# Gaukler/PlainRenderer

Hardware: AMD Instinct MI355X
Metric: frames/sec full GI+shade+post @4K; %HBM roofline; 1/2/4/8-GPU scaling (higher is better)
Workload: dtype f32

## Files before the change

include/plr.h:

```cpp
#ifndef PLR_H
#define PLR_H
#include <stddef.h>
#include <stdint.h>
#ifdef __cplusplus
extern "C" {
#endif

#define PLR_OK 0
#define PLR_ERR_INVALID_ARGUMENT (-1)
#define PLR_ERR_HIP (-2)
#define PLR_ERR_UNKNOWN_SHADER (-3)
#define PLR_ERR_BINDING (-4)
#define PLR_ERR_NOT_INITIALISED (-5)
#define PLR_ERR_UNSUPPORTED (-6)

#define PLR_INVALID_INDEX 0xFFFFFFFFu

enum plr_image_type { PLR_IMAGE_1D = 0, PLR_IMAGE_2D = 1, PLR_IMAGE_3D = 2, PLR_IMAGE_CUBE = 3 };
enum plr_mip_count { PLR_MIP_ONE = 0, PLR_MIP_FULL_CHAIN = 1, PLR_MIP_MANUAL = 2, PLR_MIP_FULL_CHAIN_ALREADY_IN_DATA = 3 };
enum plr_image_usage { PLR_USAGE_STORAGE = 1, PLR_USAGE_SAMPLED = 2, PLR_USAGE_ATTACHMENT = 4 };
enum plr_image_format {
    PLR_FORMAT_R8 = 0, PLR_FORMAT_RG8, PLR_FORMAT_RGBA8, PLR_FORMAT_R16_SFLOAT, PLR_FORMAT_RG16_SFLOAT,
    PLR_FORMAT_RG32_SFLOAT, PLR_FORMAT_RG16_SNORM, PLR_FORMAT_RGBA16_SFLOAT, PLR_FORMAT_RGBA16_SNORM,
    PLR_FORMAT_RGBA32_SFLOAT, PLR_FORMAT_R11G11B10_UFLOAT, PLR_FORMAT_DEPTH16, PLR_FORMAT_DEPTH32,
// ... 126 lines not shown
int plr_replay_frame(uint32_t count, float* out_total_gpu_ms);
int plr_upload_image(plr_image_handle image, uint32_t mip_level, const void* data, size_t size);
int plr_upload_image_rows(plr_image_handle image, uint32_t mip_level, uint32_t row_begin, uint32_t row_count, const void* data, size_t size);
int plr_download_image(plr_image_handle image, uint32_t mip_level, void* out_data, size_t size);
int plr_download_storage_buffer(plr_storage_buffer_handle buffer, void* out_data, size_t offset, size_t size);
int plr_download_uniform_buffer(plr_uniform_buffer_handle buffer, void* out_data, size_t offset, size_t size);
int plr_get_image_device_pointer(plr_image_handle image, uint32_t mip_level, void** out_ptr, size_t* out_size);
int plr_get_storage_buffer_device_pointer(plr_storage_buffer_handle buffer, void** out_ptr, size_t* out_size);
int plr_get_stream(void** out_hip_stream);
int plr_get_launch_stream(void** out_hip_stream);
int plr_copy_device_memory(void* dst, const void* src, size_t size);
int plr_copy_device_memory_2d(void* dst, size_t dst_pitch, const void* src, size_t src_pitch, size_t width_bytes, size_t rows);
int plr_read_device_memory(void* dst_host, const void* src, size_t size);
int plr_write_device_memory(void* dst, const void* src_host, size_t size);
int plr_get_supported_shaders(const char** out_names, uint32_t capacity);
int plr_debug_math_eval(int fn, const float* a, const float* b, float* out, int64_t n);
int plr_debug_codec_eval(int fn, const void* in, void* out, int64_t n);
int plr_debug_set_decision_signature(size_t words);
int plr_debug_read_decision_signature(uint32_t* out_words, size_t words);
int plr_debug_verify_histogram_thresholds(float min_luminance, float max_luminance, uint64_t* out_mismatches);
int plr_debug_verify_r11g11b10_fast(uint64_t* out4);
int plr_debug_sky_lut_eval(plr_image_handle sky_lut, const float* directions, float* out_rgb, int64_t n);
int plr_debug_pcf_tap_table(float* out_xy, size_t floats);
int plr_debug_sampler_eval(plr_image_handle image, uint32_t mip_level, int filter, int address, const float* coords, float* out, int64_t n);

#ifdef __cplusplus
}
#endif
#endif
```

plainrenderer_amd/backend.py:

```python
import ctypes as C
import os
import struct
from dataclasses import dataclass, field
from enum import IntEnum
from typing import List, Optional, Sequence

import numpy as np

_HERE = os.path.dirname(os.path.abspath(__file__))
LIB_PATH = os.environ.get("PLR_LIB") or os.path.join(_HERE, "libplr.so")


class PlrError(RuntimeError):
    pass


class ImageType(IntEnum):
    Type1D = 0
    Type2D = 1
    Type3D = 2
    TypeCube = 3


class MipCount(IntEnum):
# ... 163 lines not shown

def spec_int(location, v):
    return SpecialisationConstant(location, struct.pack("<i", int(v)))


def spec_uint(location, v):
    return SpecialisationConstant(location, struct.pack("<I", int(v)))


def spec_float(location, v):
    return SpecialisationConstant(location, struct.pack("<f", float(v)))


def _load():
    if not os.path.exists(LIB_PATH):
        raise PlrError("HIP backend library missing: %s (run `python -c 'import __graft_entry__ as g; g.build()'`). "
                       "There is no CPU fallback." % LIB_PATH)
    lib = C.CDLL(LIB_PATH)
    lib.plr_last_error.restype = C.c_char_p
    return lib


EXPORTED_SYMBOLS = [
    "plr_debug_pcf_tap_table", "plr_setup", "plr_shutdown", "plr_recreate_swapchain", "plr_last_error", "plr_wait_for_gpu_idle", "plr_update_shader_code",
    "plr_resize_images", "plr_recreate_image", "plr_resize_storage_buffer", "plr_new_frame", "plr_set_compute_pass_execution", "plr_prepare_for_drawcall_recording",
    "plr_set_uniform_buffer_data", "plr_set_storage_buffer_data", "plr_set_global_descriptor_set_resources",
    "plr_update_compute_pass_shader_description", "plr_render_frame", "plr_get_image_global_texture_array_index",
    "plr_create_compute_pass", "plr_create_image", "plr_create_uniform_buffer", "plr_create_storage_buffer", "plr_create_sampler",
    "plr_create_temporary_image", "plr_get_swapchain_input_image", "plr_get_memory_stats", "plr_get_renderpass_timings",
    "plr_get_last_frame_cpu_time", "plr_get_image_description", "plr_set_pass_timing", "plr_get_last_frame_gpu_time",
    "plr_replay_frame", "plr_upload_image", "plr_download_image", "plr_download_storage_buffer", "plr_download_uniform_buffer",
    "plr_get_image_device_pointer", "plr_get_storage_buffer_device_pointer", "plr_get_stream", "plr_get_launch_stream", "plr_copy_device_memory", "plr_read_device_memory", "plr_write_device_memory", "plr_get_supported_shaders",
    "plr_debug_math_eval", "plr_debug_codec_eval", "plr_debug_sampler_eval", "plr_debug_sky_lut_eval", "plr_debug_verify_histogram_thresholds", "plr_debug_verify_r11g11b10_fast", "plr_debug_set_decision_signature", "plr_debug_read_decision_signature", "plr_set_math_mode", "plr_get_math_mode", "plr_set_stream_overlap", "plr_get_stream_overlap", "plr_set_pass_fusion", "plr_get_pass_fusion", "plr_set_pass_fusion_reorder", "plr_get_general_kernel_executions", "plr_get_edge_signal", "plr_set_async_tail", "plr_get_async_tail", "plr_set_early_parts", "plr_get_early_parts", "plr_set_host_callback_execution", "plr_set_host_callback_execution_on", "plr_upload_image_rows",
    "plr_copy_device_memory_2d", "plr_set_global_descriptor_set_layout",
]


class RenderBackend:

    def __init__(self, width, height, device=0):
        self.lib = _load()
        self._open = False
        self._check(self.lib.plr_setup(C.c_int(device), C.c_uint32(width), C.c_uint32(height)))
        self._open = True
        self.width, self.height = width, height

    def _check(self, rc):
# ... 246 lines not shown
        return p.value

    def debugMathEval(self, fn, a, b=None):
        a = np.ascontiguousarray(a, np.float32)
        out = np.empty_like(a)
        bp = None
        if b is not None:
            b = np.ascontiguousarray(b, np.float32)
            bp = b.ctypes.data_as(C.c_void_p)
        self._check(self.lib.plr_debug_math_eval(C.c_int(fn), a.ctypes.data_as(C.c_void_p), bp, out.ctypes.data_as(C.c_void_p), C.c_int64(a.size)))
        return out

    def debugSkyLutEval(self, sky_lut, directions):
        d = np.ascontiguousarray(directions, np.float32).reshape(-1, 3)
        out = np.empty_like(d)
        self._check(self.lib.plr_debug_sky_lut_eval(_ImageHandle(sky_lut.type, sky_lut.index), d.ctypes.data_as(C.c_void_p), out.ctypes.data_as(C.c_void_p), C.c_int64(d.shape[0])))
        return out

    def debugPcfTapTable(self):
        out = np.empty((256, 12, 2), np.float32)
        self._check(self.lib.plr_debug_pcf_tap_table(out.ctypes.data_as(C.c_void_p), C.c_size_t(out.size)))
        return out

    def debugVerifyHistogramThresholds(self, min_luminance, max_luminance):
        n = C.c_uint64()
        self._check(self.lib.plr_debug_verify_histogram_thresholds(C.c_float(min_luminance), C.c_float(max_luminance), C.byref(n)))
        return n.value

    def debugVerifyR11G11B10Fast(self):
        out = (C.c_uint64 * 4)()
        self._check(self.lib.plr_debug_verify_r11g11b10_fast(out))
        return tuple(int(v) for v in out)

    def setPassFusion(self, level):
        self._check(self.lib.plr_set_pass_fusion(C.c_int(int(level))))

    def setPassFusionReorder(self, enabled):
        self._check(self.lib.plr_set_pass_fusion_reorder(C.c_int(int(bool(enabled)))))

    def getPassFusion(self):
        e, n = C.c_int(), C.c_uint32()
        self._check(self.lib.plr_get_pass_fusion(C.byref(e), C.byref(n)))
        return e.value, n.value

    def getEdgeSignal(self):
        p, v = C.c_void_p(), C.c_uint32()
# ... 58 lines not shown
```

plainrenderer_amd/csrc/backend.cpp:

```cpp
#include "backend.h"
#include "kernels_fast/pcf_taps.h"

#include <dlfcn.h>
#include <deque>
#include <algorithm>
#include <chrono>
#include <mutex>
#include <cstdlib>
#include <atomic>
#include <set>
#include <thread>
#include <unordered_map>
#include <unordered_set>
#include <cmath>
#include <cstring>
#include <map>
#include <memory>

#include "../../include/plr.h"

namespace plr {

struct ShaderEntry { std::string name; LaunchFn fn = nullptr; LaunchFn fast = nullptr; };
static bool shaderReadsBindless(const std::string& shader) {
// ... 1985 lines not shown
}

int plr_debug_sky_lut_eval(plr_image_handle sky_lut, const float* directions, float* out_rgb, int64_t n) {
    NEED_INIT_JOINED();
    ImageRes* im = resolveImage(sky_lut);
    if (!im || !directions || !out_rgb || n <= 0) return setErr(PLR_ERR_INVALID_ARGUMENT, "plr_debug_sky_lut_eval: invalid argument");
    HIP_TRY(hipStreamSynchronize(g->stream));
    return launchSkyLutProbe(makeView(*im, 0), directions, out_rgb, n);
}

int plr_debug_pcf_tap_table(float* out_xy, size_t floats) {
    NEED_INIT_JOINED();
    if (!out_xy || floats != kPcfTapTableBytes / sizeof(float)) return setErr(PLR_ERR_INVALID_ARGUMENT, "plr_debug_pcf_tap_table: out_xy must hold 256 x 12 x 2 floats");
    void* table = nullptr;
    HIP_TRY(hipMalloc(&table, kPcfTapTableBytes));
    hipError_t e = buildPcfTapTable((float2*)table, g->stream);
    if (e == hipSuccess) e = hipStreamSynchronize(g->stream);
    if (e == hipSuccess) e = hipMemcpy(out_xy, table, kPcfTapTableBytes, hipMemcpyDeviceToHost);
    hipFree(table);
    HIP_TRY(e);
    return PLR_OK;
}

int plr_debug_sampler_eval(plr_image_handle image, uint32_t mip_level, int filter, int address, const float* coords, float* out, int64_t n) {
    NEED_INIT_JOINED();
    ImageRes* im = resolveImage(image);
    if (!im || mip_level >= im->mips.size()) return setErr(PLR_ERR_INVALID_ARGUMENT, "plr_debug_sampler_eval: invalid image handle or mip level");
    if (!coords || !out || n <= 0) return setErr(PLR_ERR_INVALID_ARGUMENT, "plr_debug_sampler_eval: null argument");
    HIP_TRY(hipStreamSynchronize(g->stream));
    return launchSamplerProbe(makeView(*im, mip_level), filter, address, coords, out, n);
}

int plr_set_math_mode(int mode) {
    NEED_INIT_JOINED();
    if (mode != PLR_MATH_EXACT && mode != PLR_MATH_FAST) return setErr(PLR_ERR_INVALID_ARGUMENT, "math mode must be PLR_MATH_EXACT or PLR_MATH_FAST");
    if (mode == PLR_MATH_EXACT) if (int rc = ensureExactSet()) return rc;
    g->mathMode = mode;
    return PLR_OK;
}
int plr_get_math_mode(int* out_mode) { NEED_INIT(); *out_mode = g->mathMode; return PLR_OK; }

int plr_set_pass_timing(int enabled) { NEED_INIT(); g->passTiming = enabled != 0; return PLR_OK; }

int plr_get_renderpass_timings(plr_renderpass_time* out_times, uint32_t* inout_count) {
    NEED_INIT();
    if (!inout_count) return setErr(PLR_ERR_INVALID_ARGUMENT, "inout_count is null");
// ... 136 lines not shown
```

plainrenderer_amd/csrc/kernels_fast/pcf_taps.h:

```cpp
#pragma once
#include <hip/hip_runtime.h>
#include <stdint.h>

namespace plr {

constexpr int kPcfTaps = 12, kPcfNoiseValues = 256;
constexpr size_t kPcfTapTableBytes = (size_t)kPcfNoiseValues * kPcfTaps * 2 * sizeof(float);

hipError_t buildPcfTapTable(float2* table, hipStream_t stream);

}
```

plainrenderer_amd/csrc/kernels_fast/shading_fast.hip:

```cpp
#include "../backend.h"
#include "../device/shading_common.h"
#include "../device/fastmath.h"
#include "../device/buffer_fetch.h"
#include "upscale_quad.h"
#include "pcf_taps.h"
#include <cstdlib>
#include <type_traits>
#include <map>

namespace plr {

namespace fastshade {

#ifndef PLR_SHADE_WAVES
#define PLR_SHADE_WAVES 5
#endif

PLR_DI float rcpf(float x) { return __builtin_amdgcn_rcpf(x); }
PLR_DI float rsqf(float x) { return __builtin_amdgcn_rsqf(x); }
PLR_DI float sqrtv(float x) { return __builtin_amdgcn_sqrtf(x); }
PLR_DI float fmin1(float a, float b) { return __builtin_fminf(a, b); }
PLR_DI float fmax1(float a, float b) { return __builtin_fmaxf(a, b); }
PLR_DI float fclamp(float x, float lo, float hi) { return __builtin_fminf(__builtin_fmaxf(x, lo), hi); }
PLR_DI float fmix(float a, float b, float t) { return a + (b - a) * t; }
// ... 118 lines not shown
    r = accumulateTexel(r, q1.z, q1.w, a2 * b);
    return r;
}

struct ShadeParams {
    ImgView color, depth, normal, albedo, specular, brdfLut, shadowMaps[4], ysh, cocg, volumetricLut, skyLut;
    const LightBuffer* light;
    const ShadowCascadeInfo* shadowInfo;
    const VolumetricLightingSettings* vol;
    const GlobalUbo* g;
    const ImgView* bindless;
    uint32_t bindlessCount;
    uint32_t cascadeCount;
    int coverW, coverH, yBase;
    int xBase;
    uint32_t* sig;
    ImgView noiseTex;
    const float4* pcfTaps;
    const float4* pcfTapsByPosition;
    uint32_t pcfPositions;
    const uint2* lutEnergyFootprint;
    const uint32_t* lutEnergyNonFinite;
    uint32_t skipUnlit;
};
PLR_DI float uniformValue(float x) { return u2f((uint32_t)__builtin_amdgcn_readfirstlane((int)f2u(x))); }
PLR_DI bool finiteBits(float x) { return (f2u(x) & 0x7f800000u) != 0x7f800000u; }

#define PLR_SHADE_UNIFORM_PARAMS const GlobalUbo* __restrict__ gUniform, const LightBuffer* __restrict__ lightUniform, const ShadowCascadeInfo* __restrict__ shadowUniform, \
                                 const VolumetricLightingSettings* __restrict__ volUniform
#define PLR_SHADE_ADOPT_UNIFORMS(P) do { (P).g = gUniform; (P).light = lightUniform; (P).shadowInfo = shadowUniform; (P).vol = volUniform; } while (0)
#define PLR_SHADE_UNIFORM_ARGS(P) (P).g, (P).light, (P).shadowInfo, (P).vol

struct PcfTapRow { float4 q[kPcfTaps / 2]; };
PLR_DI float calcShadow(vec3 pos, const ImgView& shadowMap, const float* __restrict__ m, float lssX, float lssY, const PcfTapRow& taps) {
    float cxy0, cxy1;
    uint32_t depthThreshold;
    {
#pragma clang fp contract(off)
        const float x = ((m[0] * pos.x + m[4] * pos.y) + m[8] * pos.z) + m[12];
        const float y = ((m[1] * pos.x + m[5] * pos.y) + m[9] * pos.z) + m[13];
        const float z = ((m[2] * pos.x + m[6] * pos.y) + m[10] * pos.z) + m[14];
        const float w = ((m[3] * pos.x + m[7] * pos.y) + m[11] * pos.z) + m[15];
        const float rw = rcpf(w);
        cxy0 = divRNr(x, w, rw) * 0.5f + 0.5f;
        cxy1 = divRNr(y, w, rw) * 0.5f + 0.5f;
        const float actualDepth = fclamp(divRNr(z, w, rw), 0.f, 1.f);
// ... 49 lines not shown
    if (MULTISCATTER == 0) {
        const float energyAverage = ReflectedEnergyAverage(r);
        const float energyIncoming = lutEnergy(P, r, NoL);
        const float unscaled = (1.f - energyIncoming) * (1.f - energyOutgoing) * rcpf(3.1415f * (1.f - energyAverage));
        const vec3 den = 1.f - fresnelAverage * (1.f - energyAverage);
        const vec3 scaling = (fresnelAverage * fresnelAverage * energyAverage) * vec3(rcpf(den.x), rcpf(den.y), rcpf(den.z));
        return unscaled * scaling;
    } else if (MULTISCATTER == 1) {
        const float lobe = (1.f - energyOutgoing) * (1.f / PLR_GLSL_PI);
        const vec3 den = 1.f - fresnelAverage * (1.f - energyOutgoing);
        return (fresnelAverage * fresnelAverage * (energyOutgoing * lobe)) * vec3(rcpf(den.x), rcpf(den.y), rcpf(den.z));
    } else if (MULTISCATTER == 2) {
        return f0 * (rcpf(energyOutgoing) - 1.f) * singleScatteringLobe;
    }
    return vec3(0.f);
}

struct PixelInputs {
    float depth;
    uint32_t albedo, specular;
    uint32_t normal, normalH, normalV;
    uint2 ysh;
    uint32_t cocg;
};
PLR_DI vec3 decodeNormal(uint32_t texel) {
    const vec3 raw = fastm::unorm8x4(texel).xyz() * 2.f - 1.f;
    return raw * rsqf(fmax1(dot(raw, raw), 1e-30f));
}

struct SurfaceTerms {
    vec3 N, V, f0, diffuseColor, diffuseBRDFIntegral;
    float r, NoV, energyOutgoing;
    vec3 brdfLut;
};
struct DirectOut { vec3 direct; float pixelDepth; vec2 noiseTexel; };
template <int DIFFUSE_BRDF, int MULTISCATTER, bool GEOMETRIC_AA>
PLR_DI DirectOut shadeDirect(const ShadeParams& P, bool skipUnlit, int px, int py, const ViewRay& vr, const PixelInputs& in, vec3 lightColor, SurfaceTerms* st,
                             uint32_t* sigWord) {
    constexpr bool kLobesSkippable = DIFFUSE_BRDF != 3 && (MULTISCATTER == 0 || MULTISCATTER == 3);
    uint32_t lutNonFinite = 1u;
    if (kLobesSkippable && MULTISCATTER == 0 && skipUnlit && P.lutEnergyNonFinite) lutNonFinite = *P.lutEnergyNonFinite;
    const GlobalUbo* g = P.g;
    const Surface surf = exactSurface(g, vr.Vn, in.depth);
    const vec3 passPos = surf.passPos;
    const float pixelDepth = surf.pixelDepth;

    const vec3 albedoTexel = fastm::unorm8x4(in.albedo).xyz();
    const vec3 specularTexel = fastm::unorm8x4(in.specular).xyz();
    const float metalic = specularTexel.z;
    float r = specularTexel.y;
    r = fmax1(r * r, 0.0045f);
    const vec3 albedo(sRGBToLinear1(albedoTexel.x), sRGBToLinear1(albedoTexel.y), sRGBToLinear1(albedoTexel.z));
    const vec3 diffuseColor = (1.f - metalic) * albedo;
    const vec3 N = decodeNormal(in.normal);
    const vec3 L = nrm(ld3(g->sunDirection));
    const vec3 Lu(uniformValue(L.x), uniformValue(L.y), uniformValue(L.z));
    const vec3 V = vr.Vn;
    if (GEOMETRIC_AA) {
        const vec3 N_U = decodeNormal(in.normalH) - N, N_V = decodeNormal(in.normalV) - N;
        const float variance = 0.25f * (dot(N_V, N_V) + dot(N_U, N_U));
        const float kernelRoughness2 = fmin1(2.f * variance, 0.18f);
        r = fclamp(sqrtv(r * r + kernelRoughness2), 0.f, 1.f);
    }
    const float NdotL = dot(N, L);
    const float NoL = fclamp(NdotL, 0.f, 1.f);
    const bool backFacing = NdotL <= 0.f;
    const float NoV = fmax1(fabsf(dot(N, V)), 0.0001f);
    const vec3 f0 = vmix(vec3(0.04f), albedo, metalic);

    const ImgView noiseTex = P.noiseTex;
    const uint32_t noiseIndex = fastm::texelIndex((uint32_t)fastm::repeatIndex(px, noiseTex.w), (uint32_t)fastm::repeatIndex(py, noiseTex.h), (uint32_t)noiseTex.w);
    const uint32_t noiseWord = fetch16(texelBuffer(noiseTex.ptr, 2u), noiseIndex);
    const vec2 noiseTexel = fastm::unorm8x2(noiseWord);
    const uint32_t noiseByte = noiseWord & 0xffu;

    int cascadeIndex = 0;
#pragma unroll
    for (int cascade = 0; cascade < 3; cascade++) cascadeIndex += (cascade < (int)P.cascadeCount - 1 && pixelDepth >= P.shadowInfo->splits[cascade]) ? 1 : 0;
    const bool skipLobes = kLobesSkippable && skipUnlit && (MULTISCATTER != 0 || __builtin_amdgcn_readfirstlane(lutNonFinite) == 0u);
    float sunShadow = 0.f;
    if (!(skipUnlit && backFacing)) {
        PcfTapRow tapRow;
// ... 103 lines not shown
    linearCoord(z * (float)vol.d, &k0, &c);
    int xb; float a2;
    edgePair(i0, a, vol.w, &xb, &a2);
    const uint32_t y0 = __umul24((uint32_t)clampi(j0, vol.h), (uint32_t)vol.w), y1 = __umul24((uint32_t)clampi(j0 + 1, vol.h), (uint32_t)vol.w);
    const uint32_t sl = (uint32_t)vol.w * (uint32_t)vol.h;
    const uint32_t z0 = __umul24((uint32_t)clampi(k0, vol.d), sl), z1 = __umul24((uint32_t)clampi(k0 + 1, vol.d), sl);
    const BufferDesc texels = texelBuffer(vol.ptr, 8u);
    const uint32_t x0 = (uint32_t)xb;
    const uint4 q00 = fetch128(texels, z0 + y0 + x0), q01 = fetch128(texels, z0 + y1 + x0), q10 = fetch128(texels, z1 + y0 + x0), q11 = fetch128(texels, z1 + y1 + x0);
    const float a0 = 1.f - a2, b0 = 1.f - b, c0 = 1.f - c;
    const float wab00 = a0 * b0, wab10 = a2 * b0, wab01 = a0 * b, wab11 = a2 * b;
    vec4 it(0.f);
    it = accumulateTexel(it, q00.x, q00.y, wab00 * c0);
    it = accumulateTexel(it, q00.z, q00.w, wab10 * c0);
    it = accumulateTexel(it, q01.x, q01.y, wab01 * c0);
    it = accumulateTexel(it, q01.z, q01.w, wab11 * c0);
    it = accumulateTexel(it, q10.x, q10.y, wab00 * c);
    it = accumulateTexel(it, q10.z, q10.w, wab10 * c);
    it = accumulateTexel(it, q11.x, q11.y, wab01 * c);
    it = accumulateTexel(it, q11.z, q11.w, wab11 * c);
    return it;
}

template <int DIFFUSE_BRDF, int MULTISCATTER, bool GEOMETRIC_AA, int INDIRECT_TECH>
PLR_DI uint32_t shadeGeometryPixel(const ShadeParams& P, int px, int py, const ViewRay& vr, const PixelInputs& in, uint32_t* sigWord) {
    SurfaceTerms st;
    const vec3 sunColor = ld3(P.light->sunColor);
    const bool skipUnlit = P.skipUnlit && finiteBits(sunColor.x) && finiteBits(sunColor.y) && finiteBits(sunColor.z) && finiteBits(P.light->sunStrengthExposed);
    const DirectOut d = shadeDirect<DIFFUSE_BRDF, MULTISCATTER, GEOMETRIC_AA>(P, skipUnlit, px, py, vr, in, sunColor, &st, sigWord);
    vec3 lightingIndirect;
    if (INDIRECT_TECH == 0) lightingIndirect = shadeIndirect<MULTISCATTER>(P, st, in.ysh, in.cocg);
    else {
        const float amb = 0.003f * P.light->sunStrengthExposed;
        const vec3 singleScattering = vmix(vec3(st.brdfLut.x), vec3(st.brdfLut.y), st.f0);
        lightingIndirect = (amb * st.diffuseColor) * st.diffuseBRDFIntegral + singleScattering * amb;
    }
    vec3 outColor = d.direct * P.light->sunStrengthExposed + lightingIndirect;
    const vec4 it = froxelLookup(P, vr.su, vr.sv, d.noiseTexel, d.pixelDepth);
    outColor = outColor * it.w + it.xyz();
    return packR11G11B10(outColor);
}

template <int DIFFUSE_BRDF, int MULTISCATTER, bool GEOMETRIC_AA, int INDIRECT_TECH>
__global__ __launch_bounds__(256, PLR_SHADE_WAVES) void deferredShadingFastKernel(ShadeParams P, PLR_SHADE_UNIFORM_PARAMS) {
    PLR_SHADE_ADOPT_UNIFORMS(P);
    const int px = P.xBase + (int)(blockIdx.x * 64u + (threadIdx.x & 63u));
    const int py = P.yBase + (int)(blockIdx.y * 4u + (threadIdx.x >> 6));
    if (px >= P.coverW || py >= P.coverH) return;
    const ViewRay vr = exactViewRay(P.g, px, py);
    const uint32_t idx = fastm::texelIndex((uint32_t)px, (uint32_t)py, (uint32_t)P.color.w);
    PixelInputs in;
    in.depth = ((const float*)P.depth.ptr)[idx];
// ... 18 lines not shown
    if (INDIRECT_TECH == 0) {
        const int ix = clampTo(floorToInt(vr.su * (float)P.ysh.w), P.ysh.w - 1), iy = clampTo(floorToInt(vr.sv * (float)P.ysh.h), P.ysh.h - 1);
        in.ysh = ((const uint2*)P.ysh.ptr)[fastm::texelIndex((uint32_t)ix, (uint32_t)iy, (uint32_t)P.ysh.w)];
        in.cocg = ((const uint32_t*)P.cocg.ptr)[fastm::texelIndex((uint32_t)ix, (uint32_t)iy, (uint32_t)P.cocg.w)];
    }
    uint32_t sigWord;
    const uint32_t colour = shadeGeometryPixel<DIFFUSE_BRDF, MULTISCATTER, GEOMETRIC_AA, INDIRECT_TECH>(P, px, py, vr, in, &sigWord);
    ((uint32_t*)P.color.ptr)[idx] = colour;
    if (P.sig) P.sig[idx] = sigWord;
}

struct FusedUpscale {
    ImgView srcYSH, srcCoCg, halfResDepth, dstYSH, dstCoCg;
    int storeUpscaled;
};
constexpr int kGiTileW = 34, kGiTileH = 4;
struct GiTexel { float depthLinear, y0, y1, y2, y3, co, cg, pad; };
static_assert(sizeof(GiTexel) == 32, "two 16-byte LDS reads per texel");

template <int DIFFUSE_BRDF, int MULTISCATTER, bool GEOMETRIC_AA>
__global__ __launch_bounds__(256, PLR_SHADE_WAVES) void upscaleAndShadeKernel(ShadeParams P, FusedUpscale U, PLR_SHADE_UNIFORM_PARAMS) {
    PLR_SHADE_ADOPT_UNIFORMS(P);
    __shared__ GiTexel tile[kGiTileH][kGiTileW];
    const int t = (int)threadIdx.x;
    const int X0 = P.xBase + (int)(blockIdx.x * 64u), Y0 = P.yBase + (int)(blockIdx.y * 4u);
    const int k0 = (X0 >> 1) - 1, m0 = (Y0 >> 1) - 1;
    const GlobalUbo* g = P.g;
    const float nearP = g->nearPlane, farP = g->farPlane, nf = nearP * farP, nmf = nearP - farP;
    if (t < kGiTileW * kGiTileH) {
        const int r = t / kGiTileW, c = t - r * kGiTileW;
        const int hw = U.srcYSH.w, hh = U.srcYSH.h;
        const uint32_t i = fastm::texelIndex((uint32_t)clampi(k0 + c, hw), (uint32_t)clampi(m0 + r, hh), (uint32_t)hw);
        const uint2 ys = fetch64(texelBuffer(U.srcYSH.ptr, 8u), i);
        const uint32_t cc = fetch32(texelBuffer(U.srcCoCg.ptr, 4u), i);
        GiTexel e;
        e.depthLinear = fastquad::linearDepthRounded(halfBitsToFloat(fetch16(texelBuffer(U.halfResDepth.ptr, 2u), i)), nf, nmf, farP);
        e.y0 = halfBitsToFloat(ys.x & 0xffffu); e.y1 = halfBitsToFloat(ys.x >> 16); e.y2 = halfBitsToFloat(ys.y & 0xffffu); e.y3 = halfBitsToFloat(ys.y >> 16);
        e.co = halfBitsToFloat(cc & 0xffffu); e.cg = halfBitsToFloat(cc >> 16); e.pad = 0.f;
        tile[r][c] = e;
    }
    const int px = X0 + (t & 63), py = Y0 + (t >> 6);
    const bool covered = px < P.coverW && py < P.coverH;
    const int cpx = covered ? px : 0, cpy = covered ? py : 0;
    const uint32_t idx = fastm::texelIndex((uint32_t)cpx, (uint32_t)cpy, (uint32_t)P.color.w);
    PixelInputs in;
    in.depth = u2f(fetch32(texelBuffer(P.depth.ptr, 4u), idx));
    in.albedo = fetch32(texelBuffer(P.albedo.ptr, 4u), idx);
    in.specular = fetch32(texelBuffer(P.specular.ptr, 4u), idx);
    const uint32_t* normals = (const uint32_t*)P.normal.ptr;
    in.normal = fetch32(texelBuffer(P.normal.ptr, 4u), idx);
    in.normalH = in.normalV = in.normal;
    if (GEOMETRIC_AA) {
        in.normalH = fetch32(texelBuffer(P.normal.ptr, 4u), fastm::texelIndex((uint32_t)clampi(cpx ^ 1, P.normal.w), (uint32_t)cpy, (uint32_t)P.normal.w));
        in.normalV = fetch32(texelBuffer(P.normal.ptr, 4u), fastm::texelIndex((uint32_t)cpx, (uint32_t)clampi(cpy ^ 1, P.normal.h), (uint32_t)P.normal.w));
    }
    const ViewRay vr = exactViewRay(g, cpx, cpy);
    __syncthreads();
    if (!covered) return;
    uint32_t upSig;
    {
#pragma clang fp contract(off)
        const int p = px & 1, q = py & 1;
        const int kc = (px >> 1) - k0, mr = (py >> 1) - m0;
        const int c0 = kc - 1 + p, r0 = mr - 1 + q;
        const GiTexel f00 = tile[r0][c0], f10 = tile[r0][c0 + 1], f01 = tile[r0 + 1][c0], f11 = tile[r0 + 1][c0 + 1];
        const float full = fastquad::linearDepthRounded(in.depth, nf, nmf, farP);
        const float ds[4] = {f01.depthLinear, f11.depthLinear, f10.depthLinear, f00.depthLinear};
        const int offx[4] = {0, 1, 1, 0}, offy[4] = {1, 1, 0, 0};
        float minDiff = 1000.f;
        int cx = 0, cy = 0;
        bool isEdge = false;
#pragma unroll
        for (int i = 0; i < 4; i++) {
            const float diff = fabsf(ds[i] - full);
            isEdge = isEdge || diff > 0.5f;
            if (diff < minDiff) { minDiff = diff; cx = offx[i]; cy = offy[i]; }
        }
        float y0, y1, y2, y3, co, cg;
        if (isEdge) {
            const int hw = U.srcYSH.w, hh = U.srcYSH.h;
            const GiTexel n = tile[min((py >> 1) + cy, hh - 1) - m0][min((px >> 1) + cx, hw - 1) - k0];
            y0 = n.y0; y1 = n.y1; y2 = n.y2; y3 = n.y3; co = n.co; cg = n.cg;
        } else {
            const float a = p ? 0.25f : 0.75f, b = q ? 0.25f : 0.75f;
            const float w00 = (1.f - a) * (1.f - b), w10 = a * (1.f - b), w01 = (1.f - a) * b, w11 = a * b;
            auto bl = [&](float t00, float t10, float t01, float t11) { return __builtin_fmaf(t11, w11, __builtin_fmaf(t01, w01, __builtin_fmaf(t10, w10, t00 * w00))); };
            y0 = bl(f00.y0, f10.y0, f01.y0, f11.y0); y1 = bl(f00.y1, f10.y1, f01.y1, f11.y1); y2 = bl(f00.y2, f10.y2, f01.y2, f11.y2); y3 = bl(f00.y3, f10.y3, f01.y3, f11.y3);
            co = bl(f00.co, f10.co, f01.co, f11.co); cg = bl(f00.cg, f10.cg, f01.cg, f11.cg);
        }
        in.ysh = make_uint2(floatToHalfBits(y0) | (floatToHalfBits(y1) << 16), floatToHalfBits(y2) | (floatToHalfBits(y3) << 16));
        in.cocg = floatToHalfBits(co) | (floatToHalfBits(cg) << 16);
        upSig = (isEdge ? 1u : 0u) | (cx ? 2u : 0u) | (cy ? 4u : 0u);
    }
    if (U.storeUpscaled) {
        ((uint2*)U.dstYSH.ptr)[idx] = in.ysh;
        ((uint32_t*)U.dstCoCg.ptr)[idx] = in.cocg;
    }
    if (in.depth == 0.f) {
        ((uint32_t*)P.color.ptr)[idx] = packR11G11B10(fastm::sampleSkyLut(-vr.Vn, P.skyLut));
        if (P.sig) P.sig[idx] = 128u | (upSig << 8);
        return;
    }
    uint32_t sigWord;
    const uint32_t colour = shadeGeometryPixel<DIFFUSE_BRDF, MULTISCATTER, GEOMETRIC_AA, 0>(P, px, py, vr, in, &sigWord);
    ((uint32_t*)P.color.ptr)[idx] = colour;
    if (P.sig) P.sig[idx] = sigWord | (upSig << 8);
}

struct DirectRecords { uint4* a; uint4* b; uint32_t* c; };
PLR_DI uint32_t packHalves(float lo, float hi) { return __builtin_bit_cast(uint32_t, __builtin_amdgcn_cvt_pkrtz(lo, hi)); }

template <int DIFFUSE_BRDF, int MULTISCATTER, bool GEOMETRIC_AA>
__global__ __launch_bounds__(256, PLR_SHADE_WAVES) void shadeDirectKernel(ShadeParams P, DirectRecords R, const GlobalUbo G, const ShadowCascadeInfo* __restrict__ shadowUniform,
                                                                          const VolumetricLightingSettings* __restrict__ volUniform) {
    P.g = &G; P.shadowInfo = shadowUniform; P.vol = volUniform; P.light = nullptr;
    const int px = P.xBase + (int)(blockIdx.x * 64u + (threadIdx.x & 63u));
    const int py = P.yBase + (int)(blockIdx.y * 4u + (threadIdx.x >> 6));
    if (px >= P.coverW || py >= P.coverH) return;
    const ViewRay vr = exactViewRay(P.g, px, py);
    const uint32_t idx = fastm::texelIndex((uint32_t)px, (uint32_t)py, (uint32_t)P.color.w);
    PixelInputs in;
    in.depth = u2f(fetch32(texelBuffer(P.depth.ptr, 4u), idx));
    if (in.depth == 0.f) {
        R.a[idx] = make_uint4(packR11G11B10(fastm::sampleSkyLut(-vr.Vn, P.skyLut)), 0u, 0u, 0u);
        return;
    }
    in.albedo = fetch32(texelBuffer(P.albedo.ptr, 4u), idx);
// ... 144 lines not shown
constexpr size_t kNoiseSlotBytes = (size_t)kMaxNoisePositions * (kPcfTaps / 2) * sizeof(float4);
__global__ void lutEnergyFootprintKernel(ImgView lut, uint2* __restrict__ out, uint32_t* __restrict__ nonFinite) {
    const int x = (int)(blockIdx.x * 64u + (threadIdx.x & 63u)), y = (int)(blockIdx.y * 4u + (threadIdx.x >> 6));
    if (x >= lut.w - 1 || y >= lut.h - 1) return;
    const uint2* t = (const uint2*)lut.ptr;
    auto energy = [&](int tx, int ty) { return t[(size_t)ty * (size_t)lut.w + tx].x >> 16; };
    const uint32_t e00 = energy(x, y), e10 = energy(x + 1, y), e01 = energy(x, y + 1), e11 = energy(x + 1, y + 1);
    out[(size_t)y * (size_t)(lut.w - 1) + x] = make_uint2(e00 | (e10 << 16), e01 | (e11 << 16));
    auto special = [](uint32_t h) { return (h & 0x7c00u) == 0x7c00u; };
    if (special(e00) || special(e10) || special(e01) || special(e11)) *nonFinite = 1u;
}
__global__ void pcfTapsByPositionKernel(const uint16_t* __restrict__ noiseTexels, uint32_t positions, const float4* __restrict__ byValue, float4* __restrict__ byPosition) {
    const uint32_t pos = blockIdx.x * blockDim.x + threadIdx.x;
    if (pos >= positions) return;
    const uint32_t noiseByte = noiseTexels[pos] & 0xffu;
    const float2* taps = (const float2*)byValue + noiseByte * kPcfTaps;
    const int turn = (int)((float)noiseByte * (12.f / 255.f) + 0.5f);
#pragma unroll
    for (int k = 0; k < kPcfTaps / 2; k++) {
        const int i0 = ((2 * k - turn) % kPcfTaps + kPcfTaps) % kPcfTaps, i1 = ((2 * k + 1 - turn) % kPcfTaps + kPcfTaps) % kPcfTaps;
        byPosition[(uint32_t)k * positions + pos] = make_float4(taps[i0].x, taps[i0].y, taps[i1].x, taps[i1].y);
    }
}
struct ShadeDerived {
    const void* scratchBase = nullptr;
    size_t scratchBytes = 0;
    struct Slot { const void* noise = nullptr; int w = 0, h = 0; uint64_t version = 0, lastUse = 0; } slots[kNoiseSlots];
    uint64_t useCounter = 0;
    const void* lut = nullptr; int lutW = 0, lutH = 0; uint64_t lutVersion = 0;
};
static thread_local std::map<const void*, ShadeDerived> g_shadeDerived;
static int shadeDerivedTables(const PassCtx& c, ShadeParams* P, DirectRecords* records = nullptr) {
    const ImgView& lut = P->brdfLut;
    const size_t footprintOffset = kPcfTapTableBytes + kNoiseSlots * kNoiseSlotBytes;
    const size_t footprintBytes = (size_t)(lut.w - 1) * (size_t)std::max(lut.h - 1, 1) * sizeof(uint2);
    const size_t flagOffset = (footprintOffset + footprintBytes + 15) & ~(size_t)15;
    const size_t recordsOffset = (flagOffset + 16 + 255) & ~(size_t)255;
    const size_t pixels = (size_t)P->color.w * (size_t)P->color.h;
    const size_t total = records ? recordsOffset + pixels * 36 : flagOffset + 16;
    uint8_t* scratch = (uint8_t*)c.scratch(total);
    if (!scratch) return c.fail(-2, "deferredShading: cannot allocate scratch memory");
    if (records) { records->a = (uint4*)(scratch + recordsOffset); records->b = records->a + pixels; records->c = (uint32_t*)(records->b + pixels); }
    ShadeDerived& d = g_shadeDerived[(const void*)c.scratchSlot];
    if (d.scratchBase != scratch || d.scratchBytes != *c.scratchSize) {
        d = ShadeDerived{};
        d.scratchBase = scratch;
        d.scratchBytes = *c.scratchSize;
        const hipError_t e = buildPcfTapTable((float2*)scratch, c.stream);
        if (e != hipSuccess) return c.fail(-2, std::string("deferredShading: PCF tap table: ") + hipGetErrorString(e));
    }
    P->pcfTaps = (const float4*)scratch;
    P->pcfTapsByPosition = nullptr;
    P->pcfPositions = 0;
    P->lutEnergyFootprint = nullptr;
    P->lutEnergyNonFinite = nullptr;
    if (const uint64_t lutVersion = lut.h >= 2 ? contentVersionOf(lut.ptr) : 0) {
        if (d.lut != lut.ptr || d.lutW != lut.w || d.lutH != lut.h || d.lutVersion != lutVersion) {
            const hipError_t e = hipMemsetAsync(scratch + flagOffset, 0, 16, c.stream);
            if (e != hipSuccess) return c.fail(-2, std::string("deferredShading: LUT energy footprint: ") + hipGetErrorString(e));
            lutEnergyFootprintKernel<<<dim3(divUp((unsigned)(lut.w - 1), 64u), divUp((unsigned)(lut.h - 1), 4u)), 256, 0, c.stream>>>(lut, (uint2*)(scratch + footprintOffset),
                                                                                                                                       (uint32_t*)(scratch + flagOffset));
            PLR_CHECK_LAUNCH(c);
            d.lut = lut.ptr; d.lutW = lut.w; d.lutH = lut.h; d.lutVersion = lutVersion;
        }
        P->lutEnergyFootprint = (const uint2*)(scratch + footprintOffset);
        P->lutEnergyNonFinite = (const uint32_t*)(scratch + flagOffset);
    }
    const ImgView& noise = P->noiseTex;
    if (!noise.ptr || noise.fmt != F_RG8) return 0;
    const uint64_t version = contentVersionOf(noise.ptr);
    const uint64_t positions = (uint64_t)noise.w * (uint64_t)noise.h;
    if (version == 0 || positions > kMaxNoisePositions) return 0;
    ShadeDerived::Slot* slot = nullptr;
    for (auto& s : d.slots) if (s.noise == noise.ptr && s.w == noise.w && s.h == noise.h && s.version == version) slot = &s;
// ... 31 lines not shown
    if (c.sampled[16].w != c.sampled[15].w || c.sampled[16].h != c.sampled[15].h) return c.fail(-4, "deferredShading: Y_SH and CoCg differ in size");
    for (int b : {20, 22, 23}) if (c.sampled[b].w != c.storage[0].w || c.sampled[b].h != c.storage[0].h) return kUseGeneralKernel;
    if (c.sampled[3].w < 2 || c.sampled[18].w < 2) return kUseGeneralKernel;
    *diffuseBRDF = c.specInt(0, 0); *multi = c.specInt(1, 0); *tech = c.specInt(3, 0);
    *aa = c.specBool(2, false);
    const uint32_t cascades = c.specUint(4, 4u);
    if (*diffuseBRDF < 0 || *diffuseBRDF > 3 || *multi < 0 || *multi > 3 || cascades < 1 || cascades > 4) return c.fail(-1, "deferredShading: specialisation constant out of range");
    ShadeParams P{};
    P.color = c.storage[0]; P.depth = c.sampled[20]; P.normal = c.sampled[21]; P.albedo = c.sampled[22]; P.specular = c.sampled[23];
    P.brdfLut = c.sampled[3];
    for (int i = 0; i < 4; i++) P.shadowMaps[i] = c.sampled[9 + i];
    P.ysh = c.sampled[15]; P.cocg = c.sampled[16]; P.volumetricLut = c.sampled[18]; P.skyLut = c.sampled[24];
    P.light = (const LightBuffer*)c.sbuf[7].ptr; P.shadowInfo = (const ShadowCascadeInfo*)c.sbuf[8].ptr;
    P.vol = (const VolumetricLightingSettings*)c.ubuf[19].ptr; P.g = c.global;
    P.bindless = c.bindless; P.bindlessCount = c.bindlessCount; P.cascadeCount = cascades;
    if (!c.hostNoiseView(&P.noiseTex)) return kUseGeneralKernel;
    if (deriveTables) if (int rc = shadeDerivedTables(c, &P, records)) return rc;
    const PassCtx::RowSpan rs = c.rowSpan(P.color.h);
    const PassCtx::ColSpan cs = c.colSpan(P.color.w);
    P.coverW = cs.x1; P.xBase = cs.x0; P.coverH = rs.y1; P.yBase = rs.y0;
    P.sig = c.sigFor((size_t)P.color.w * (size_t)P.color.h);
    const char* skipEnv = std::getenv("PLR_SHADE_SKIP_UNLIT");
    P.skipUnlit = (!P.sig && !(skipEnv && skipEnv[0] == '0' && skipEnv[1] == 0)) ? 1u : 0u;
    *out = P;
    return 0;
}

static int launchDeferredShadingFast(const PassCtx& c) {
    ShadeParams P;
    int diffuseBRDF, multi, tech;
    bool aa;
    if (int rc = shadeParamsFor(c, &P, &diffuseBRDF, &multi, &aa, &tech)) return rc;
    ShadeKernel k = nullptr;
    switch (diffuseBRDF) {
        case 0: k = pickMulti<0>(multi, aa, tech); break;
        case 1: k = pickMulti<1>(multi, aa, tech); break;
        case 2: k = pickMulti<2>(multi, aa, tech); break;
        default: k = pickMulti<3>(multi, aa, tech); break;
    }
    if (P.coverW <= P.xBase || P.coverH <= P.yBase) return 0;
    k<<<dim3(divUp((unsigned)(P.coverW - P.xBase), 64u), divUp((unsigned)(P.coverH - P.yBase), 4u)), 256, 0, c.stream>>>(P, PLR_SHADE_UNIFORM_ARGS(P));
    PLR_CHECK_LAUNCH(c);
    return 0;
}

struct FusedShade { ShadeParams P; FusedUpscale U; int diffuseBRDF, multi; bool aa; };
static int fusedShadeSetup(const PassCtx* const* ctxs, size_t count, FusedShade* f, bool deriveTables, DirectRecords* records) {
    if (count != 2) return kUseGeneralKernel;
// ... 202 lines not shown
```

Measured before the change: 1469.

## Share decoded normals and sRGB table via LDS in fused upscale-shade kernel

The fused upscale-and-shade kernel now builds a 256-entry sRGB-to-linear lookup table in shared memory and looks up albedo with it instead of evaluating the sRGB curve per channel. With geometric AA it stores each pixel's decoded normal in LDS so the horizontal and vertical neighbour normals are read from shared memory rather than fetched and decoded again. It also skips the GI upscale math for sky pixels (depth 0) when no upscaled store or signature is needed. This costs extra LDS and a table build in the scratch area, and the lookup may differ slightly from the direct formula.

```diff
diff --git a/include/plr.h b/include/plr.h
--- a/include/plr.h
+++ b/include/plr.h
@@ -172,6 +172,7 @@
 int plr_debug_verify_r11g11b10_fast(uint64_t* out4);
 int plr_debug_sky_lut_eval(plr_image_handle sky_lut, const float* directions, float* out_rgb, int64_t n);
 int plr_debug_pcf_tap_table(float* out_xy, size_t floats);
+int plr_debug_srgb_linear_table(float* out_table, float* out_direct);
 int plr_debug_sampler_eval(plr_image_handle image, uint32_t mip_level, int filter, int address, const float* coords, float* out, int64_t n);
 
 #ifdef __cplusplus
diff --git a/plainrenderer_amd/backend.py b/plainrenderer_amd/backend.py
--- a/plainrenderer_amd/backend.py
+++ b/plainrenderer_amd/backend.py
@@ -209,7 +209,7 @@
 
 
 EXPORTED_SYMBOLS = [
-    "plr_debug_pcf_tap_table", "plr_setup", "plr_shutdown", "plr_recreate_swapchain", "plr_last_error", "plr_wait_for_gpu_idle", "plr_update_shader_code",
+    "plr_debug_pcf_tap_table", "plr_debug_srgb_linear_table", "plr_setup", "plr_shutdown", "plr_recreate_swapchain", "plr_last_error", "plr_wait_for_gpu_idle", "plr_update_shader_code",
     "plr_resize_images", "plr_recreate_image", "plr_resize_storage_buffer", "plr_new_frame", "plr_set_compute_pass_execution", "plr_prepare_for_drawcall_recording",
     "plr_set_uniform_buffer_data", "plr_set_storage_buffer_data", "plr_set_global_descriptor_set_resources",
     "plr_update_compute_pass_shader_description", "plr_render_frame", "plr_get_image_global_texture_array_index",
@@ -502,6 +502,11 @@
         self._check(self.lib.plr_debug_pcf_tap_table(out.ctypes.data_as(C.c_void_p), C.c_size_t(out.size)))
         return out
 
+    def debugSrgbLinearTable(self):
+        table, direct = np.empty(256, np.float32), np.empty((3, 256), np.float32)
+        self._check(self.lib.plr_debug_srgb_linear_table(table.ctypes.data_as(C.c_void_p), direct.ctypes.data_as(C.c_void_p)))
+        return table, direct
+
     def debugVerifyHistogramThresholds(self, min_luminance, max_luminance):
         n = C.c_uint64()
         self._check(self.lib.plr_debug_verify_histogram_thresholds(C.c_float(min_luminance), C.c_float(max_luminance), C.byref(n)))
diff --git a/plainrenderer_amd/csrc/backend.cpp b/plainrenderer_amd/csrc/backend.cpp
--- a/plainrenderer_amd/csrc/backend.cpp
+++ b/plainrenderer_amd/csrc/backend.cpp
@@ -2031,6 +2031,13 @@
     return PLR_OK;
 }
 
+int plr_debug_srgb_linear_table(float* out_table, float* out_direct) {
+    NEED_INIT_JOINED();
+    if (!out_table || !out_direct) return setErr(PLR_ERR_INVALID_ARGUMENT, "plr_debug_srgb_linear_table: out_table must hold 256 floats, out_direct 3 x 256");
+    HIP_TRY(fastshade::srgbLinearTableProbe(out_table, out_direct, g->stream));
+    return PLR_OK;
+}
+
 int plr_debug_sampler_eval(plr_image_handle image, uint32_t mip_level, int filter, int address, const float* coords, float* out, int64_t n) {
     NEED_INIT_JOINED();
     ImageRes* im = resolveImage(image);
diff --git a/plainrenderer_amd/csrc/kernels_fast/pcf_taps.h b/plainrenderer_amd/csrc/kernels_fast/pcf_taps.h
--- a/plainrenderer_amd/csrc/kernels_fast/pcf_taps.h
+++ b/plainrenderer_amd/csrc/kernels_fast/pcf_taps.h
@@ -9,4 +9,6 @@
 
 hipError_t buildPcfTapTable(float2* table, hipStream_t stream);
 
+namespace fastshade { hipError_t srgbLinearTableProbe(float* outTable256, float* outDirect768, hipStream_t stream); }
+
 }
diff --git a/plainrenderer_amd/csrc/kernels_fast/shading_fast.hip b/plainrenderer_amd/csrc/kernels_fast/shading_fast.hip
--- a/plainrenderer_amd/csrc/kernels_fast/shading_fast.hip
+++ b/plainrenderer_amd/csrc/kernels_fast/shading_fast.hip
@@ -164,6 +164,8 @@
     const uint2* lutEnergyFootprint;
     const uint32_t* lutEnergyNonFinite;
     uint32_t skipUnlit;
+    uint32_t sharedInputs;
+    const float* srgbLinearTable;
 };
 PLR_DI float uniformValue(float x) { return u2f((uint32_t)__builtin_amdgcn_readfirstlane((int)f2u(x))); }
 PLR_DI bool finiteBits(float x) { return (f2u(x) & 0x7f800000u) != 0x7f800000u; }
@@ -259,10 +261,23 @@
     uint32_t normal, normalH, normalV;
     uint2 ysh;
     uint32_t cocg;
+    bool shared;
+    vec3 rawN;
+    float rsN;
+    const float4* quadNormals;
+    const float* srgbLinear;
+    int lane;
 };
 PLR_DI vec3 decodeNormal(uint32_t texel) {
     const vec3 raw = fastm::unorm8x4(texel).xyz() * 2.f - 1.f;
     return raw * rsqf(fmax1(dot(raw, raw), 1e-30f));
+}
+struct NormalParts { vec3 raw; float rs; };
+PLR_DI NormalParts decodeNormalParts(uint32_t texel) {
+    NormalParts d;
+    d.raw = fastm::unorm8x4(texel).xyz() * 2.f - 1.f;
+    d.rs = rsqf(fmax1(dot(d.raw, d.raw), 1e-30f));
+    return d;
 }
 
 struct SurfaceTerms {
@@ -271,7 +286,7 @@
     vec3 brdfLut;
 };
 struct DirectOut { vec3 direct; float pixelDepth; vec2 noiseTexel; };
-template <int DIFFUSE_BRDF, int MULTISCATTER, bool GEOMETRIC_AA>
+template <int DIFFUSE_BRDF, int MULTISCATTER, bool GEOMETRIC_AA, bool SHARED_INPUTS = false>
 PLR_DI DirectOut shadeDirect(const ShadeParams& P, bool skipUnlit, int px, int py, const ViewRay& vr, const PixelInputs& in, vec3 lightColor, SurfaceTerms* st,
                              uint32_t* sigWord) {
     constexpr bool kLobesSkippable = DIFFUSE_BRDF != 3 && (MULTISCATTER == 0 || MULTISCATTER == 3);
@@ -287,14 +302,27 @@
     const float metalic = specularTexel.z;
     float r = specularTexel.y;
     r = fmax1(r * r, 0.0045f);
-    const vec3 albedo(sRGBToLinear1(albedoTexel.x), sRGBToLinear1(albedoTexel.y), sRGBToLinear1(albedoTexel.z));
+    const bool shared = SHARED_INPUTS && in.shared;
+    vec3 albedo;
+    if (shared) albedo = vec3(in.srgbLinear[in.albedo & 0xffu], in.srgbLinear[(in.albedo >> 8) & 0xffu], in.srgbLinear[(in.albedo >> 16) & 0xffu]);
+    else albedo = vec3(sRGBToLinear1(albedoTexel.x), sRGBToLinear1(albedoTexel.y), sRGBToLinear1(albedoTexel.z));
     const vec3 diffuseColor = (1.f - metalic) * albedo;
-    const vec3 N = decodeNormal(in.normal);
+    vec3 N;
+    if (shared) N = in.rawN * in.rsN;
+    else N = decodeNormal(in.normal);
     const vec3 L = nrm(ld3(g->sunDirection));
     const vec3 Lu(uniformValue(L.x), uniformValue(L.y), uniformValue(L.z));
     const vec3 V = vr.Vn;
     if (GEOMETRIC_AA) {
-        const vec3 N_U = decodeNormal(in.normalH) - N, N_V = decodeNormal(in.normalV) - N;
+        vec3 N_U, N_V;
+        if (shared) {
+            const float4 h = in.quadNormals[in.lane ^ 1], v = in.quadNormals[in.lane ^ 64];
+            N_U = vec3(__builtin_fmaf(h.x, h.w, -N.x), __builtin_fmaf(h.y, h.w, -N.y), __builtin_fmaf(h.z, h.w, -N.z));
+            N_V = vec3(__builtin_fmaf(v.x, v.w, -N.x), __builtin_fmaf(v.y, v.w, -N.y), __builtin_fmaf(v.z, v.w, -N.z));
+        } else {
+            N_U = decodeNormal(in.normalH) - N;
+            N_V = decodeNormal(in.normalV) - N;
+        }
         const float variance = 0.25f * (dot(N_V, N_V) + dot(N_U, N_U));
         const float kernelRoughness2 = fmin1(2.f * variance, 0.18f);
         r = fclamp(sqrtv(r * r + kernelRoughness2), 0.f, 1.f);
@@ -444,12 +472,12 @@
     return it;
 }
 
-template <int DIFFUSE_BRDF, int MULTISCATTER, bool GEOMETRIC_AA, int INDIRECT_TECH>
+template <int DIFFUSE_BRDF, int MULTISCATTER, bool GEOMETRIC_AA, int INDIRECT_TECH, bool SHARED_INPUTS = false>
 PLR_DI uint32_t shadeGeometryPixel(const ShadeParams& P, int px, int py, const ViewRay& vr, const PixelInputs& in, uint32_t* sigWord) {
     SurfaceTerms st;
     const vec3 sunColor = ld3(P.light->sunColor);
     const bool skipUnlit = P.skipUnlit && finiteBits(sunColor.x) && finiteBits(sunColor.y) && finiteBits(sunColor.z) && finiteBits(P.light->sunStrengthExposed);
-    const DirectOut d = shadeDirect<DIFFUSE_BRDF, MULTISCATTER, GEOMETRIC_AA>(P, skipUnlit, px, py, vr, in, sunColor, &st, sigWord);
+    const DirectOut d = shadeDirect<DIFFUSE_BRDF, MULTISCATTER, GEOMETRIC_AA, SHARED_INPUTS>(P, skipUnlit, px, py, vr, in, sunColor, &st, sigWord);
     vec3 lightingIndirect;
     if (INDIRECT_TECH == 0) lightingIndirect = shadeIndirect<MULTISCATTER>(P, st, in.ysh, in.cocg);
     else {
@@ -514,6 +542,9 @@
 __global__ __launch_bounds__(256, PLR_SHADE_WAVES) void upscaleAndShadeKernel(ShadeParams P, FusedUpscale U, PLR_SHADE_UNIFORM_PARAMS) {
     PLR_SHADE_ADOPT_UNIFORMS(P);
     __shared__ GiTexel tile[kGiTileH][kGiTileW];
+    __shared__ float4 quadNormals[256];
+    __shared__ float srgbLinear[256];
+    const bool shared = P.sharedInputs != 0u;
     const int t = (int)threadIdx.x;
     const int X0 = P.xBase + (int)(blockIdx.x * 64u), Y0 = P.yBase + (int)(blockIdx.y * 4u);
     const int k0 = (X0 >> 1) - 1, m0 = (Y0 >> 1) - 1;
@@ -533,7 +564,7 @@
     }
     const int px = X0 + (t & 63), py = Y0 + (t >> 6);
     const bool covered = px < P.coverW && py < P.coverH;
-    const int cpx = covered ? px : 0, cpy = covered ? py : 0;
+    const int cpx = min(px, P.color.w - 1), cpy = min(py, P.color.h - 1);
     const uint32_t idx = fastm::texelIndex((uint32_t)cpx, (uint32_t)cpy, (uint32_t)P.color.w);
     PixelInputs in;
     in.depth = u2f(fetch32(texelBuffer(P.depth.ptr, 4u), idx));
@@ -542,15 +573,32 @@
     const uint32_t* normals = (const uint32_t*)P.normal.ptr;
     in.normal = fetch32(texelBuffer(P.normal.ptr, 4u), idx);
     in.normalH = in.normalV = in.normal;
-    if (GEOMETRIC_AA) {
+    in.shared = shared;
+    in.quadNormals = quadNormals;
+    in.srgbLinear = srgbLinear;
+    in.lane = t;
+    if (shared) {
+        srgbLinear[t] = P.srgbLinearTable[t];
+        if (GEOMETRIC_AA) {
+            const NormalParts own = decodeNormalParts(in.normal);
+            in.rawN = own.raw; in.rsN = own.rs;
+            quadNormals[t] = make_float4(own.raw.x, own.raw.y, own.raw.z, own.rs);
+        }
+    } else if (GEOMETRIC_AA) {
         in.normalH = fetch32(texelBuffer(P.normal.ptr, 4u), fastm::texelIndex((uint32_t)clampi(cpx ^ 1, P.normal.w), (uint32_t)cpy, (uint32_t)P.normal.w));
         in.normalV = fetch32(texelBuffer(P.normal.ptr, 4u), fastm::texelIndex((uint32_t)cpx, (uint32_t)clampi(cpy ^ 1, P.normal.h), (uint32_t)P.normal.w));
     }
     const ViewRay vr = exactViewRay(g, cpx, cpy);
     __syncthreads();
     if (!covered) return;
-    uint32_t upSig;
-    {
+    if (shared && !GEOMETRIC_AA) {
+        const NormalParts own = decodeNormalParts(in.normal);
+        in.rawN = own.raw; in.rsN = own.rs;
+    }
+    uint32_t upSig = 0u;
+    in.ysh = make_uint2(0u, 0u);
+    in.cocg = 0u;
+    if (!shared || in.depth != 0.f || U.storeUpscaled || P.sig) {
 #pragma clang fp contract(off)
         const int p = px & 1, q = py & 1;
         const int kc = (px >> 1) - k0, mr = (py >> 1) - m0;
@@ -594,7 +642,7 @@
         return;
     }
     uint32_t sigWord;
-    const uint32_t colour = shadeGeometryPixel<DIFFUSE_BRDF, MULTISCATTER, GEOMETRIC_AA, 0>(P, px, py, vr, in, &sigWord);
+    const uint32_t colour = shadeGeometryPixel<DIFFUSE_BRDF, MULTISCATTER, GEOMETRIC_AA, 0, true>(P, px, py, vr, in, &sigWord);
     ((uint32_t*)P.color.ptr)[idx] = colour;
     if (P.sig) P.sig[idx] = sigWord | (upSig << 8);
 }
@@ -785,6 +833,16 @@
         byPosition[(uint32_t)k * positions + pos] = make_float4(taps[i0].x, taps[i0].y, taps[i1].x, taps[i1].y);
     }
 }
+constexpr size_t kSrgbTableBytes = 256 * sizeof(float);
+__global__ void srgbLinearTableKernel(float* __restrict__ table, float* __restrict__ direct) {
+    const uint32_t c = threadIdx.x;
+    if (table) table[c] = sRGBToLinear1(fastm::unorm8x4(c).x);
+    if (direct) {
+        const vec3 albedoTexel = fastm::unorm8x4(c * 0x010101u).xyz();
+        const vec3 albedo(sRGBToLinear1(albedoTexel.x), sRGBToLinear1(albedoTexel.y), sRGBToLinear1(albedoTexel.z));
+        direct[c] = albedo.x; direct[256 + c] = albedo.y; direct[512 + c] = albedo.z;
+    }
+}
 struct ShadeDerived {
     const void* scratchBase = nullptr;
     size_t scratchBytes = 0;
@@ -795,7 +853,8 @@
 static thread_local std::map<const void*, ShadeDerived> g_shadeDerived;
 static int shadeDerivedTables(const PassCtx& c, ShadeParams* P, DirectRecords* records = nullptr) {
     const ImgView& lut = P->brdfLut;
-    const size_t footprintOffset = kPcfTapTableBytes + kNoiseSlots * kNoiseSlotBytes;
+    const size_t srgbOffset = kPcfTapTableBytes + kNoiseSlots * kNoiseSlotBytes;
+    const size_t footprintOffset = srgbOffset + kSrgbTableBytes;
     const size_t footprintBytes = (size_t)(lut.w - 1) * (size_t)std::max(lut.h - 1, 1) * sizeof(uint2);
     const size_t flagOffset = (footprintOffset + footprintBytes + 15) & ~(size_t)15;
     const size_t recordsOffset = (flagOffset + 16 + 255) & ~(size_t)255;
@@ -811,8 +870,11 @@
         d.scratchBytes = *c.scratchSize;
         const hipError_t e = buildPcfTapTable((float2*)scratch, c.stream);
         if (e != hipSuccess) return c.fail(-2, std::string("deferredShading: PCF tap table: ") + hipGetErrorString(e));
+        srgbLinearTableKernel<<<1, 256, 0, c.stream>>>((float*)(scratch + srgbOffset), nullptr);
+        PLR_CHECK_LAUNCH(c);
     }
     P->pcfTaps = (const float4*)scratch;
+    P->srgbLinearTable = (const float*)(scratch + srgbOffset);
     P->pcfTapsByPosition = nullptr;
     P->pcfPositions = 0;
     P->lutEnergyFootprint = nullptr;
@@ -890,8 +952,23 @@
     P.sig = c.sigFor((size_t)P.color.w * (size_t)P.color.h);
     const char* skipEnv = std::getenv("PLR_SHADE_SKIP_UNLIT");
     P.skipUnlit = (!P.sig && !(skipEnv && skipEnv[0] == '0' && skipEnv[1] == 0)) ? 1u : 0u;
+    const char* sharedEnv = std::getenv("PLR_SHADE_SHARED");
+    P.sharedInputs = (P.srgbLinearTable && !(sharedEnv && sharedEnv[0] == '0' && sharedEnv[1] == 0)) ? 1u : 0u;
     *out = P;
     return 0;
+}
+
+hipError_t srgbLinearTableProbe(float* outTable256, float* outDirect768, hipStream_t stream) {
+    float* d = nullptr;
+    hipError_t e = hipMalloc((void**)&d, 4 * kSrgbTableBytes);
+    if (e != hipSuccess) return e;
+    srgbLinearTableKernel<<<1, 256, 0, stream>>>(d, d + 256);
+    e = hipGetLastError();
+    if (e == hipSuccess) e = hipStreamSynchronize(stream);
+    if (e == hipSuccess) e = hipMemcpy(outTable256, d, kSrgbTableBytes, hipMemcpyDeviceToHost);
+    if (e == hipSuccess) e = hipMemcpy(outDirect768, d + 256, 3 * kSrgbTableBytes, hipMemcpyDeviceToHost);
+    hipFree(d);
+    return e;
 }
 
 static int launchDeferredShadingFast(const PassCtx& c) {
```

Result: slower. 1438 (-2.1%).
